# maxrmorrison/promonet

Hardware: AMD Instinct MI355X
Metric: audio samples/sec (22.05 kHz), batch-32 10 s utterances (higher is better)
Workload: dtype bf16; 1 GPU; Generator.forward (prepare_features + HiFi-GAN), batch 32 x 10 s per GPU (861 frames, 220416 samples each), random-init weights, bf16 MFMA operands, fp32 accumulate and activations; model=hifigan, batch_per_gpu=32, frames=861, devices=1, parallelism=batch-sharded x1

## Files before the change

### include/promonet_hip.h

```cpp
#ifndef PROMONET_HIP_H
#define PROMONET_HIP_H

#include <stddef.h>
#include <stdint.h>

#ifdef __cplusplus
extern "C" {
#endif

#define PM_OK 0
#define PM_EINVAL (-1)
#define PM_ESTATE (-2)
#define PM_EHIP (-3)
#define PM_ENOMEM (-4)
#define PM_ETIMEOUT (-5)

#define PM_F32 0
#define PM_F16 1
#define PM_BF16 2
#define PM_F16X3 3
#define PM_F16A2 4
#define PM_F16UX 5

#define PM_MAX_STAGES 8
// ... 49 lines not shown
                              void* stream);

int pm_hifigan_context(pm_hifigan_t h, int* left, int* right);
int pm_hifigan_stream(pm_hifigan_t h, const float* chunk, int chunk_cl,
                      int chunk_frames, const float* prev_window,
                      int prev_frames, int keep, float* next_window,
                      const float* global_features, int global_batch,
                      int emit_first, int emit_frames, float* out, int batch,
                      void* workspace, size_t workspace_bytes, void* stream);
size_t pm_hifigan_stream_workspace_bytes(pm_hifigan_t h, int batch,
                                         int window_frames);

int pm_hifigan_profile_enable(pm_hifigan_t h, int enable);
int pm_hifigan_profile_only(pm_hifigan_t h, const char* label);
int pm_hifigan_profile_collect(pm_hifigan_t h);
int pm_hifigan_profile_reset(pm_hifigan_t h);
const char* pm_hifigan_profile_report(pm_hifigan_t h);

#define PM_SPARSE_NONE 0
#define PM_SPARSE_PERCENTILE 1
#define PM_SPARSE_CONSTANT 2
#define PM_SPARSE_TOPK 3
int pm_prepare_features(const float* loudness, const float* pitch,
                        const float* periodicity, const float* ppg,
                        const float* pitch_edges, const float* pitch_table,
                        float* out_ref, float* out_cl, int batch, int frames,
                        int loudness_rows, int ppg_channels, int pitch_bins,
                        int embedding_size, int bands, int cl_channels,
                        int sparse_method, float ppg_threshold, float fmin,
                        float fmax, float min_db, float ref_db,
                        float period_rate, void* stream);

int pm_prepare_global_features(const int64_t* speakers,
                               const float* spectral_balance_ratios,
                               const float* loudness_ratios,
                               const float* speaker_table, float* out,
                               int batch, int speaker_channels,
                               int num_speakers, void* stream);
int pm_prepare_global_features_linear(const float* speaker_embeddings,
                                      const float* weight, const float* bias,
                                      const float* spectral_balance_ratios,
                                      const float* loudness_ratios,
                                      float* out, int batch,
                                      int embedding_channels,
                                      int speaker_channels, void* stream);

size_t pm_op_workspace_bytes(int c_in, int c_out, int k);
int pm_block_iteration_cl(int dtype, const float* x_cl, float* out_cl,
                          const float* w1, const float* b1, const float* w2,
                          const float* b2, int batch, int length,
                          int channels, int kernel_size, int dilation,
                          int mode, float scale, void* workspace,
                          size_t workspace_bytes, void* stream);
int pm_block_cl(int dtype, const float* x_cl, float* out_cl,
                const float* const* w1, const float* const* b1,
                const float* const* w2, const float* const* b2,
                const int* dilations, int niter, int batch, int length,
                int channels, int kernel_size, int mode, float scale,
                void* workspace, size_t workspace_bytes, void* stream);
int pm_block_act16_cl(int dtype, int act_dtype, const float* x_cl,
                      float* out_cl, void* act16_cl, const float* const* w1,
                      const float* const* b1, const float* const* w2,
                      const float* const* b2, const int* dilations, int niter,
                      int batch, int length, int channels, int kernel_size,
                      int mode, float scale, void* workspace,
                      size_t workspace_bytes, void* stream);
int pm_mrf_cl(int dtype, const float* x_cl, float* out_cl,
              const float* const* w1, const float* const* b1,
              const float* const* w2, const float* const* b2,
              const int* dilations, int niter, int batch, int length,
              int channels, void* workspace, size_t workspace_bytes,
              void* stream);
int pm_input_conv_cl(int dtype, const float* x_cl, float* out_cl,
                     const float* weight, const float* bias,
                     const float* global_features,
                     const float* speaker_weight, const float* speaker_bias,
                     int global_batch, int global_channels, int batch,
                     int length, int c_in, int c_out, void* workspace,
                     size_t workspace_bytes, void* stream);
int pm_conv_transpose_cl(int dtype, const float* x_cl, float* out_cl,
                         const float* w, const float* bias, int batch,
                         int length, int c_in, int c_out, int rate, int lrelu,
                         void* workspace, size_t workspace_bytes,
                         void* stream);
int pm_conv_transpose_ragged_cl(int dtype, const float* x_cl, float* out_cl,
                                const float* w, const float* bias,
                                const int* lengths, int batch, int length,
                                int c_in, int c_out, int rate, int lrelu,
                                void* workspace, size_t workspace_bytes,
                                void* stream);
int pm_conv_transpose_x16_cl(int dtype, const void* x16_cl, float* out_cl,
                             const float* w, const float* bias, int batch,
                             int length, int c_in, int c_out, int rate,
                             void* workspace, size_t workspace_bytes,
                             void* stream);
int pm_out_conv_tanh(const float* x_cl, const float* w, float* out,
                     int batch, int length, int channels, void* stream);
int pm_debug_timeline(void* dev_buffer);
int pm_debug_force(int walk_nseg, int upsample_groups);
int pm_debug_skew(int mode);
int pm_mfma_probe(int dtype, int iterations, const void* operands,
                  float* sink, int workgroups, void* stream);
size_t pm_walk_scratch_bytes(int batch);
int pm_fold_weight_norm(const float* g, const float* v, float* w, int rows,
                        int cols, void* stream);
int pm_to_channels_last(const float* src, float* dst, int batch, int channels,
// ... 336 lines not shown
```

### promonet_amd/_lib.py

```python
import ctypes
import os
from pathlib import Path

import torch

LIB_PATH = Path(__file__).parent / 'lib' / 'libpromonet_hip.so'

PM_F32, PM_F16, PM_BF16, PM_F16X3, PM_F16A2, PM_F16UX = 0, 1, 2, 3, 4, 5
DTYPES = {'fp32': PM_F32, 'f32': PM_F32, 'f16': PM_F16, 'fp16': PM_F16,
          'bf16': PM_BF16, 'f16x3': PM_F16X3, 'f16a2': PM_F16A2,
          'f16ux': PM_F16UX,
          'mixed': 16}
MAX_STAGES, MAX_RESBLOCKS, MAX_DILATIONS = 8, 4, 4
SPARSE_METHODS = {None: 0, 'percentile': 1, 'constant': 2, 'topk': 3}
DISC_SPEC_R, DISC_SPEC_CMB, DISC_SPEC_DB = range(3)
FDISC_ACTIVATIONS = {'none': 0, 'relu': 1, 'sigmoid': 2}
(ADV_ABS_DIFF, ADV_SQ_ONE_MINUS, ADV_SQ, ADV_HINGE_ONE_MINUS,
 ADV_HINGE_ONE_PLUS) = range(5)
(OPTIM_MAX, OPTIM_MIN, OPTIM_MEAN, OPTIM_NORM, OPTIM_NORM_SQ, OPTIM_NONFINITE,
 OPTIM_FOUND_INF, OPTIM_INV_SCALE, OPTIM_COEF) = range(9)
OPTIM_STATS = 16

c_float_p = ctypes.c_void_p
c_int64_p = ctypes.POINTER(ctypes.c_int64)


class HifiganConfig(ctypes.Structure):
    _fields_ = [
        ('num_features', ctypes.c_int),
        ('global_channels', ctypes.c_int),
        ('initial_channels', ctypes.c_int),
        ('num_stages', ctypes.c_int),
        ('upsample_rates', ctypes.c_int * MAX_STAGES),
        ('upsample_kernel_sizes', ctypes.c_int * MAX_STAGES),
        ('num_resblocks', ctypes.c_int),
        ('resblock_kernel_sizes', ctypes.c_int * MAX_RESBLOCKS),
        ('num_dilations', ctypes.c_int),
        ('resblock_dilations', (ctypes.c_int * MAX_DILATIONS) * MAX_RESBLOCKS),
        ('compute_dtype', ctypes.c_int),
        ('stage_compute_dtype', ctypes.c_int * MAX_STAGES)]


_I, _F, _P, _S = ctypes.c_int, ctypes.c_float, ctypes.c_void_p, ctypes.c_size_t
_D = ctypes.c_double
SIGNATURES = {
    'pm_version': (_I, []),
    'pm_last_error': (ctypes.c_char_p, []),
    'pm_hifigan_create': (_I, [ctypes.POINTER(HifiganConfig),
                               ctypes.POINTER(_P)]),
    'pm_hifigan_destroy': (_I, [_P]),
    'pm_hifigan_load_tensor': (_I, [_P, ctypes.c_char_p, _P, c_int64_p, _I, _P]),
    'pm_hifigan_finalize': (_I, [_P, _P]),
    'pm_hifigan_workspace_bytes': (_S, [_P, _I, _I]),
    'pm_hifigan_hopsize': (_I, [_P]),
    'pm_hifigan_features_cl_channels': (_I, [_P]),
    'pm_hifigan_forward': (_I, [_P, _P, _P, _I, _P, _I, _I, _P, _S, _P]),
    'pm_hifigan_forward_cl': (_I, [_P, _P, _P, _I, _P, _I, _I, _P, _S, _P]),
    'pm_hifigan_forward_ragged': (_I, [_P, _P, _I, _P, _I, _P, _P, _I, _I, _P, _S, _P]),
    'pm_hifigan_context': (_I, [_P, ctypes.POINTER(_I), ctypes.POINTER(_I)]),
    'pm_hifigan_stream': (_I, [_P, _P, _I, _I, _P, _I, _I, _P, _P, _I, _I, _I,
                               _P, _I, _P, _S, _P]),
    'pm_hifigan_stream_workspace_bytes': (_S, [_P, _I, _I]),
    'pm_hifigan_profile_enable': (_I, [_P, _I]),
    'pm_hifigan_profile_only': (_I, [_P, ctypes.c_char_p]),
    'pm_hifigan_profile_collect': (_I, [_P]),
    'pm_hifigan_profile_reset': (_I, [_P]),
    'pm_hifigan_profile_report': (ctypes.c_char_p, [_P]),
    'pm_prepare_features': (_I, [_P] * 8 + [_I] * 9 + [_F] * 6 + [_P]),
    'pm_prepare_global_features': (_I, [_P] * 5 + [_I, _I, _I, _P]),
    'pm_prepare_global_features_linear': (_I, [_P] * 6 + [_I, _I, _I, _P]),
    'pm_op_workspace_bytes': (_S, [_I, _I, _I]),
    'pm_block_iteration_cl': (_I, [_I] + [_P] * 6 + [_I] * 6 + [_F, _P, _S, _P]),
    'pm_block_cl': (_I, [_I, _P, _P] + [_P] * 5 + [_I] * 6 + [_F, _P, _S, _P]),
    'pm_block_act16_cl': (
        _I, [_I, _I, _P, _P, _P] + [_P] * 5 + [_I] * 6 + [_F, _P, _S, _P]),
    'pm_mrf_cl': (_I, [_I, _P, _P] + [_P] * 5 + [_I] * 4 + [_P, _S, _P]),
    'pm_input_conv_cl': (_I, [_I] + [_P] * 7 + [_I] * 6 + [_P, _S, _P]),
    'pm_conv_transpose_cl': (_I, [_I] + [_P] * 4 + [_I] * 6 + [_P, _S, _P]),
    'pm_conv_transpose_ragged_cl': (
        _I, [_I] + [_P] * 5 + [_I] * 6 + [_P, _S, _P]),
    'pm_conv_transpose_x16_cl': (_I, [_I] + [_P] * 4 + [_I] * 5 + [_P, _S, _P]),
    'pm_out_conv_tanh': (_I, [_P, _P, _P, _I, _I, _I, _P]),
    'pm_debug_timeline': (_I, [_P]),
    'pm_debug_force': (_I, [_I, _I]),
    'pm_debug_skew': (_I, [_I]),
    'pm_mfma_probe': (_I, [_I, _I, _P, _P, _I, _P]),
    'pm_walk_scratch_bytes': (_S, [_I]),
    'pm_fold_weight_norm': (_I, [_P, _P, _P, _I, _I, _P]),
    'pm_to_channels_last': (_I, [_P, _P, _I, _I, _I, _I, _P]),
    'pm_grid_sample': (_I, [_P, _P, _P, _I, _I, _I, _I, _F, _F, _F, _F, _P]),
    'pm_stretch_grid': (_I, [_P, _I, _P, _I, _P, _P, _I, _I, _P]),
    'pm_fargan_create': (_I, [_I, _I, _I, ctypes.POINTER(_P)]),
    'pm_fargan_destroy': (_I, [_P]),
    'pm_fargan_load_tensor': (_I, [_P, ctypes.c_char_p, _P, c_int64_p, _I, _P]),
    'pm_fargan_finalize': (_I, [_P, _P]),
    'pm_fargan_workspace_bytes': (_S, [_P, _I, _I]),
    'pm_fargan_forward': (_I, [_P, _P, _I, _P, _I, _P, _I, _P, _I, _I, _P, _S, _P]),
    'pm_fargan_forward_ragged': (_I, [_P, _P, _I, _P, _I, _P, _I, _P, _P, _I, _I, _P, _S, _P]),
    'pm_fargan_forward_stateful': (_I, [_P, _P, _I, _P, _I, _P, _I, _P, _P, _P, _P, _I, _I, _P, _S, _P]),
    'pm_fargan_set_mode': (_I, [_P, _I]),
    'pm_fargan_check': (_I, [_P, _I, _I, _P, _P]),
    'pm_stft_scratch_bytes': (_S, [_I, _I]),
    'pm_stft_magnitude': (_I, [_P, _P, _I, _I, _P, _S, _P]),
    'pm_stft_magnitude_dft': (_I, [_P, _P, _I, _I, _P, _S, _P]),
    'pm_stft_mel_scratch_bytes': (_S, [_I]),
    'pm_stft_mel_prepare': (_I, [_P, _I, _P, _S, _P]),
    'pm_stft_mel': (_I, [_P, _P, _P, _I, _I, _I, _I, _F, _P]),
    'pm_stft_set_frames_per_group': (_I, [_I]),
    'pm_stft_set_loudness_passes': (_I, [_I]),
    'pm_stft_launch_info': (_I, [_I, _I, _I, ctypes.POINTER(_I), ctypes.POINTER(_I)]),
    'pm_linear_to_mel': (_I, [_P, _P, _P, _I, _I, _I, _I, _I, _F, _P]),
    'pm_stft_backward_scratch_bytes': (_S, [_I, _I]),
    'pm_stft_magnitude_backward': (_I, [_P, _P, _P, _I, _I, _P, _S, _P]),
    'pm_linear_to_mel_backward': (_I, [_P] * 5 + [_I] * 5 + [_F, _P]),
    'pm_loudness_scratch_bytes': (_S, [_I, _I]),
    'pm_loudness': (_I, [_P, _P, _P, _I, _I, _I, _F, _P, _S, _P]),
    'pm_limit_tile': (_I, [ctypes.POINTER(_I), ctypes.POINTER(_I)]),
    'pm_limit_workspace_bytes': (_S, [_I]),
    'pm_limit': (_I, [_P] * 4 + [_I, _I, ctypes.c_int64, ctypes.c_int64, _I] +
                 [_F] * 4 + [_P, _S, _P]),
    'pm_loudness_shift': (_I, [_P] * 5 + [_I, _I, ctypes.c_int64, _I,
                                          ctypes.c_int64, ctypes.c_int64, _P]),
    'pm_resample_tile': (_I, [_I, _I, _I]),
    'pm_resample': (_I, [_P, _P, _P, _P, _I, _I, ctypes.c_int64, _I, _I, _I, _I,
                         ctypes.c_int64, _P]),
# ... 134 lines not shown
```

### promonet_amd/csrc/pm_api.hip

```cpp
#include <hip/hip_runtime.h>

#include <algorithm>
#include <cstdarg>
#include <cstdio>
#include <cstring>
#include <map>
#include <mutex>
#include <string>
#include <vector>

#include "pm_host.h"
#include "pm_launch.h"
#include "pm_misc.h"

#define PM_VERSION 100

static thread_local char g_error[512] = "";

int pm_fail(int code, const char* fmt, ...) {
    va_list ap;
    va_start(ap, fmt);
    vsnprintf(g_error, sizeof(g_error), fmt, ap);
    va_end(ap);
    return code;
// ... 973 lines not shown
    if (!speakers || !table || !out) return pm_fail(PM_EINVAL, "null argument");
    if (B < 1 || S < 1 || num_speakers < 1)
        return pm_fail(PM_EINVAL, "bad dimensions");
    hipLaunchKernelGGL(pm_global_features_kernel, dim3(B), dim3(256), 0,
                       (hipStream_t)stream, (const long long*)speakers, sbr,
                       lr, table, out, B, S, num_speakers);
    PM_HIP_TRY(hipGetLastError());
    return PM_OK;
}

extern "C" int pm_prepare_global_features_linear(
    const float* emb, const float* weight, const float* bias,
    const float* sbr, const float* lr, float* out, int B, int E, int S,
    void* stream) {
    if (!emb || !weight || !bias || !out)
        return pm_fail(PM_EINVAL, "null argument");
    if (B < 1 || E < 1 || S < 1) return pm_fail(PM_EINVAL, "bad dimensions");
    hipLaunchKernelGGL(pm_global_features_linear_kernel,
                       dim3((S + 3) / 4, B), dim3(256), 0,
                       (hipStream_t)stream, emb, weight, bias, sbr, lr, out, B,
                       E, S);
    PM_HIP_TRY(hipGetLastError());
    return PM_OK;
}

struct IterationLayout { float *w1, *w2, *b1, *b2; size_t total; };
static IterationLayout iteration_layout(int c_in, int c_out, int k,
                                        void* base) {
    const size_t ci = pm_pad32(c_in), co = pm_pad32(c_out);
    PmCarve c(base);
    return {c.take<float>(ci * co * k + co * 16),
            c.take<float>(ci * co * k + co * 16), c.take<float>(co * 64),
            c.take<float>(co * 64), c.used};
}

extern "C" size_t pm_op_workspace_bytes(int c_in, int c_out, int k) {
    return iteration_layout(c_in, c_out, k, nullptr).total;
}

static int pack_iteration(
    int dtype, int C, int K, const float* w1, const float* b1, const float* w2,
    const float* b2, char* base, hipStream_t s, const void** p1,
    const void** p2) {
    const IterationLayout l = iteration_layout(C, C, K, base);
    Layer conv = mrf_layer(dtype, C, K);
    conv.w = l.w1; conv.bias = l.b1;
    PM_HIP_TRY(pack_layer(conv, w1, b1, s));
    conv.w = l.w2; conv.bias = l.b2;
    PM_HIP_TRY(pack_layer(conv, w2, b2, s));
    *p1 = l.w1; *p2 = l.w2;
    return PM_OK;
}

extern "C" int pm_block_iteration_cl(
    int dtype, const float* x, float* out, const float* w1, const float* b1,
    const float* w2, const float* b2, int B, int L, int C, int K, int d,
    int mode, float scale, void* ws, size_t ws_bytes, void* stream) {
    if (!x || !out || !w1 || !b1 || !w2 || !b2 || !ws)
        return pm_fail(PM_EINVAL, "null argument");
    const int Cp = pm_pad32(C);
    if (Cp != 32 && Cp != 64 && Cp != 128 && Cp != 256)
        return pm_fail(PM_EINVAL, "channels %d unsupported", C);
    if ((K != 3 && K != 7 && K != 11) || d < 1 || d > 5)
        return pm_fail(PM_EINVAL, "kernel %d / dilation %d unsupported", K, d);
    if (ws_bytes < pm_op_workspace_bytes(C, C, K))
        return pm_fail(PM_ENOMEM, "workspace too small");
    hipStream_t s = (hipStream_t)stream;
    const void *p1, *p2;
    const int rc = pack_iteration(dtype, C, K, w1, b1, w2, b2, (char*)ws, s,
                                  &p1, &p2);
    if (rc) return rc;
    PairArgs a = {};
    a.x = x; a.out = out; a.w1 = p1; a.w2 = p2;
    a.B = B; a.L = L; a.dilation = d; a.mode = mode; a.scale = scale;
    PM_HIP_TRY(launch_pair(dtype, Cp, K, a, s));
    return PM_OK;
}

extern "C" int pm_debug_timeline(void* dev_buffer) {
#ifdef PM_TUNING
    g_timeline = (unsigned long long*)dev_buffer;
    return PM_OK;
#else
    (void)dev_buffer;
    return pm_fail(PM_ESTATE, "pm_debug_timeline needs a -DPM_TUNING build "
                              "(make TUNING=1)");
#endif
}

static int block_cl_impl(
    int dtype, const float* x, float* out, const float* const* w1,
    const float* const* b1, const float* const* w2, const float* const* b2,
    const int* dilations, int niter, int B, int L, int C, int K, int mode,
    float scale, void* ws, size_t ws_bytes, void* stream, void* act16,
    int act_dtype) {
    if (!x || !out || !w1 || !b1 || !w2 || !b2 || !dilations || !ws)
        return pm_fail(PM_EINVAL, "null argument");
    const int Cp = pm_pad32(C);
    if (Cp > 256)
        return pm_fail(PM_EINVAL, "channels %d unsupported (<= 256)", C);
    if ((K != 3 && K != 7 && K != 11) || niter < 1 || niter > 3)
        return pm_fail(PM_EINVAL,
                       "kernel %d / %d iterations unsupported", K, niter);
    const size_t per = iteration_layout(C, C, K, nullptr).total;
    if (ws_bytes < 3 * per)
        return pm_fail(PM_ENOMEM, "workspace too small");
    hipStream_t s = (hipStream_t)stream;
    PmStage d = stage_desc(Cp, x, out, B, L, mode, scale, 1, niter);
    d.blk[0].K = K;
    for (int n = 0; n < niter; ++n) {
        const int rc = pack_iteration(dtype, C, K, w1[n], b1[n], w2[n], b2[n],
                                      (char*)ws + n * per, s, &d.blk[0].w1[n],
                                      &d.blk[0].w2[n]);
        if (rc) return rc;
        d.blk[0].dil[n] = dilations[n];
    }
    if (ws_bytes > 3 * per) {
        d.scratch = (char*)ws + 3 * per;
        d.scratch_bytes = ws_bytes - 3 * per;
    }
    if (act16) { d.act16 = act16; d.act16_type = act_dtype; }
    PmPlan plan;
    PM_HIP_TRY(plan_stage(dtype, d, 1, &plan));
    if (plan.block[0].kernel == PM_PAIRS)
        return pm_fail(PM_EINVAL, "no whole-Block kernel for this shape");
    PM_HIP_TRY(launch_block3(dtype, plan.block[0], d, 0, s));
    if (act16 && !plan.block[0].act16)
        return pm_fail(PM_ESTATE,
                       "the launch did not take the skewed walk: `out` "
// ... 292 lines not shown
```

### promonet_amd/csrc/pm_conv.h

```cpp
#pragma once
#include <type_traits>

#include "pm_common.h"


template <class ET, int CH, int NT, int XR_MAX>
struct ChunkStager {
    static constexpr int Q = CH / 4;
    static constexpr int MAXIT = (XR_MAX * Q + NT - 1) / NT;
    static constexpr int S = CH * ET::ESZ + 16;
    float4 r[MAXIT];

    __device__ __forceinline__ void load(
        const float* __restrict__ xb, int cstride, int c0, int t_first,
        int XR, int L, int tid) {
        const int lo = max(t_first, 0);
        const int hi = min(L, t_first + XR);
        const __amdgpu_buffer_rsrc_t rsrc = __builtin_amdgcn_make_buffer_rsrc(
            const_cast<float*>(xb) + (size_t)lo * cstride, 0,
            max(hi - lo, 0) * cstride * 4, 0x00020000);
#pragma unroll
        for (int it = 0; it < MAXIT; ++it) {
            const int idx = tid + it * NT;
            const int row = idx / Q, q = idx % Q;
// ... 341 lines not shown
#pragma unroll
        for (int g4 = 0; g4 < 4; g4 += 2) {
            float4 lo = pm_lrelu4(acc_quad(v, g4));
            float4 hi = pm_lrelu4(acc_quad(v, g4 + 1));
            if (MASK && zero) {
                lo = make_float4(0.f, 0.f, 0.f, 0.f);
                hi = lo;
            }
            uint2 a = ET::pack4(lo), b = ET::pack4(hi);
            auto sx = __builtin_amdgcn_permlane32_swap(a.x, b.x, false, false);
            auto sy = __builtin_amdgcn_permlane32_swap(a.y, b.y, false, false);
            *reinterpret_cast<uint4*>(rowp + (ch + 8 * (g4 + lh)) * 2) =
                make_uint4(sx[0], sy[0], sx[1], sy[1]);
        }
    } else if constexpr (ET::SPLIT && !PM_SPLIT_STORE8) {
#pragma unroll
        for (int g4 = 0; g4 < 4; ++g4) {
            float4 q = pm_lrelu4(acc_quad(v, g4));
            if (MASK && zero) q = make_float4(0.f, 0.f, 0.f, 0.f);
            half4 hi, lo;
            ElemF16X3::split4(q, hi, lo);
            const uint2 a = __builtin_bit_cast(uint2, hi);
            const uint2 b = __builtin_bit_cast(uint2, lo);
            auto sx = __builtin_amdgcn_permlane32_swap(a.x, b.x, false, false);
            auto sy = __builtin_amdgcn_permlane32_swap(a.y, b.y, false, false);
            *reinterpret_cast<uint4*>(rowp + ((ch >> 3) + g4) * 32 + lh * 16) =
                make_uint4(sx[0], sy[0], sx[1], sy[1]);
        }
    } else {
#pragma unroll
        for (int g4 = 0; g4 < 4; ++g4) {
            float4 q = pm_lrelu4(acc_quad(v, g4));
            if (MASK && zero) q = make_float4(0.f, 0.f, 0.f, 0.f);
            ET::store4_at(rowp, ch + 8 * g4 + 4 * lh, q);
        }
    }
}

template <class ET>
__device__ __forceinline__ void store_tile_lrelu(
    char* rowp, const int ch, const floatx16& v, const int t_tile,
    const int L, const int ln, const int lh) {
#if defined(PM_TUNING) && defined(PM_ABLATE_EPI)
    return;
#endif
    if (t_tile >= 0 && t_tile + 32 <= L) {
        store_tile_lrelu_impl<ET, false>(rowp, ch, v, false, lh);
    } else {
        const int t = t_tile + ln;
        store_tile_lrelu_impl<ET, true>(rowp, ch, v, !(t >= 0 && t < L), lh);
    }
}


struct PairArgs {
    const float* x;
    float* out;
    const void* w1;
    const void* w2;
    int B, L;
    int dilation;
    int mode;
    float scale;
    int ntiles;
    const int* lengths;
    int len_scale;
    PM_TIMELINE_FIELD
};

template <int C, int K, int WN, int NTW>
struct PairGeom {
    static constexpr int N1 = WN * NTW * 32;
    static constexpr int TL = N1 - (K - 1);
};

template <class ET, int C, int K, int WM, int WN, int NTW, int CH, int ALIAS>
__host__ __device__ constexpr int pair_smem_bytes(int d) {
    constexpr int NCH = C / CH;
    constexpr int N1 = WN * NTW * 32;
    const int x = (NCH > 1 ? 2 : 1) * (N1 + (K - 1) * d) * (CH * ET::ESZ + 16);
    const int inter = (N1 + K - 1) * (C * ET::ESZ + 16);
    return ALIAS ? (x > inter ? x : inter) : x + inter;
}

template <class ET, int C, int K, int WM, int WN, int NTW, int CH, int ALIAS>
__global__ __launch_bounds__(WM * WN * 64) void conv_pair_kernel(
    PairArgs a) {
    typedef typename ET::afrag_t frag_t;
    constexpr int NCH = C / CH;
    constexpr int KC = CH / 16;
    constexpr int MT = C / 32;
    constexpr int MTW = MT / WM;
    static_assert(MT % WM == 0, "WM must divide the M tile count");
    constexpr int N1 = WN * NTW * 32;
    constexpr int NT = WM * WN * 64;
    constexpr int H2 = (K - 1) / 2;
    constexpr int TL = N1 - (K - 1);
    constexpr int SX = CH * ET::ESZ + 16;
    constexpr int SI = C * ET::ESZ + 16;
    constexpr int XR_MAX = N1 + (K - 1) * 5;
    constexpr int G = (ET::ESZ == 4) ? (KC >= 2 ? 2 : 1)
                    : (KC < 4 ? KC : (NTW >= 6 && K == 11 ? 2 : 4));

    extern __shared__ __attribute__((aligned(16))) char smem[];

    const int tid = threadIdx.x;
// ... 65 lines not shown
        if (more) {
            pm_block_sync();
            if (c < 2) PM_STAMP(a, 8 + 3 * c);
        }
    }

    PM_STAMP(a, 2);
    if (ALIAS) pm_block_sync();
    load_bias_frags<ET, MTW>(bf, w2 + W_BIAS, W_MT_STRIDE);
#pragma unroll
    for (int mt = 0; mt < MTW; ++mt) {
#pragma unroll
        for (int nt = 0; nt < NTW; ++nt) {
            const int n_first = (wn * NTW + nt) * 32;
            const int n = n_first + ln;
            const int t_tile = t0 - H2 + n_first;
            store_tile_lrelu<ET>(inter + n * SI, (wm * MTW + mt) * 32,
                                 acc[mt][nt], t_tile, L, ln, lh);
            const int t = min(t0 + n, L - 1);
            const float* xr = xb + (size_t)t * C +
                              (wm * MTW + mt) * 32 + 4 * lh;
#pragma unroll
            for (int g4 = 0; g4 < 4; ++g4) {
                const float4 r = *reinterpret_cast<const float4*>(xr + 8 * g4);
                acc[mt][nt][4 * g4 + 0] = r.x;
                acc[mt][nt][4 * g4 + 1] = r.y;
                acc[mt][nt][4 * g4 + 2] = r.z;
                acc[mt][nt][4 * g4 + 3] = r.w;
            }
        }
    }
    pm_block_sync();
    __builtin_amdgcn_sched_barrier(0);
    bias_add<ET, MTW, NTW>(acc, bf);
    PM_STAMP(a, 3);

    const int lane_off_i = ((wn * NTW * 32) + ln) * SI + lh * 8 * ET::ESZ;
#pragma unroll 1
    for (int c = 0; c < NCH; ++c) {
        mma_taps<ET, K, KC, MTW, NTW, G, SI>(
            acc, inter + lane_off_i + c * CH * ET::ESZ, SI,
            w2 + (size_t)c * W_CHUNK, W_MT_STRIDE, afirst,
            c + 1 < NCH ? w2 + (size_t)(c + 1) * W_CHUNK : nullptr);
    }

    PM_STAMP(a, 4);
    const int mode = a.mode;
    const float scale = a.scale;
    const int rows = min(TL, L - t0);
    const __amdgpu_buffer_rsrc_t orsrc = __builtin_amdgcn_make_buffer_rsrc(
        a.out + ((size_t)b * a.L + t0) * C, 0, rows * C * 4, 0x00020000);
    const unsigned voff0 =
        (unsigned)(((wn * NTW * 32 + ln) * C + wm * MTW * 32 + 4 * lh) * 4);
    if (mode == 2) {
        constexpr int NB = NTW > 4 ? (NTW + 1) / 2 : NTW;
#pragma unroll
        for (int mt = 0; mt < MTW; ++mt)
#pragma unroll
            for (int n0 = 0; n0 < NTW; n0 += NB) {
                pm_u4 old[NB][4];
#pragma unroll
                for (int i = 0; i < NB; ++i) {
                    if (n0 + i >= NTW) break;
                    const unsigned voff =
                        voff0 + (unsigned)((mt * 32 + (n0 + i) * 32 * C) * 4);
#pragma unroll
                    for (int g4 = 0; g4 < 4; ++g4)
                        old[i][g4] = __builtin_amdgcn_raw_buffer_load_b128(
                            orsrc, voff + g4 * 32, 0, 0);
                }
#pragma unroll
                for (int i = 0; i < NB; ++i) {
                    if (n0 + i >= NTW) break;
                    const int nt = n0 + i;
                    const unsigned voff =
                        voff0 + (unsigned)((mt * 32 + nt * 32 * C) * 4);
#pragma unroll
                    for (int g4 = 0; g4 < 4; ++g4) {
                        const pm_u4 o = old[i][g4];
                        pm_u4 r;
                        r.x = __float_as_uint(__uint_as_float(o.x) +
                                              acc[mt][nt][4 * g4 + 0] * scale);
                        r.y = __float_as_uint(__uint_as_float(o.y) +
                                              acc[mt][nt][4 * g4 + 1] * scale);
                        r.z = __float_as_uint(__uint_as_float(o.z) +
                                              acc[mt][nt][4 * g4 + 2] * scale);
                        r.w = __float_as_uint(__uint_as_float(o.w) +
                                              acc[mt][nt][4 * g4 + 3] * scale);
                        __builtin_amdgcn_raw_buffer_store_b128(
                            r, orsrc, voff + g4 * 32, 0, 0);
                    }
                }
            }
    } else {
        const float s = mode == 1 ? scale : 1.f;
#pragma unroll
        for (int mt = 0; mt < MTW; ++mt)
#pragma unroll
            for (int nt = 0; nt < NTW; ++nt) {
                const unsigned voff =
                    voff0 + (unsigned)((mt * 32 + nt * 32 * C) * 4);
#pragma unroll
                for (int g4 = 0; g4 < 4; ++g4) {
                    pm_u4 r;
                    r.x = __float_as_uint(acc[mt][nt][4 * g4 + 0] * s);
                    r.y = __float_as_uint(acc[mt][nt][4 * g4 + 1] * s);
                    r.z = __float_as_uint(acc[mt][nt][4 * g4 + 2] * s);
                    r.w = __float_as_uint(acc[mt][nt][4 * g4 + 3] * s);
                    __builtin_amdgcn_raw_buffer_store_b128(
                        r, orsrc, voff + g4 * 32, 0, 0);
                }
            }
    }
    PM_STAMP(a, 5);
    PM_STAMP_WALL(a, blockIdx.x, 13);
}


#ifndef PM_ROWS_AUX
#define PM_ROWS_AUX 2
#endif
#ifndef PM_SINGLE_ROWS
#define PM_SINGLE_ROWS 1
#endif
template <int MTW, int CP>
struct RowStores {
    static constexpr int RUN = MTW * 32 * 4;
    static constexpr int WAVE = CP * RUN;
    static constexpr int LPR = RUN / 16;
    static constexpr int CPI = 64 / LPR;
    static_assert(MTW == 1 || MTW == 2, "8 or 16 slots of 16 bytes");
    static_assert(CP == 8 || CP == 16 || CP == 32, "whole 8-lane store groups");
    static __device__ __forceinline__ int at(int col, int s) {
        return col * RUN + ((s ^ (col & 7)) << 4);
    }
};

template <int MTW, int NTW, int CP>
__device__ __forceinline__ void pm_store_rows(
    const floatx16 (&acc)[MTW][NTW], char* ebuf, const float* bias_ptr,
    const float* gb, __amdgpu_buffer_rsrc_t orsrc, int M, int m0, int n0,
    int lane) {
    typedef RowStores<MTW, CP> R;
    const int ln = lane & 31, lh = lane >> 5;
    const int q = lane % R::LPR, h = lane / R::LPR;
    const int co = m0 + 4 * q;
    float4 bias = *reinterpret_cast<const float4*>(bias_ptr + co);
    if (gb) {
        const float4 g = *reinterpret_cast<const float4*>(gb + co);
        bias.x += g.x; bias.y += g.y; bias.z += g.z; bias.w += g.w;
    }
#pragma unroll
    for (int pass = 0; pass < NTW * (32 / CP); ++pass) {
        const int nt = pass / (32 / CP), sub = pass % (32 / CP);
        pm_wave_lds_sync();
        if (CP == 32 || ln / CP == sub) {
#pragma unroll
            for (int mt = 0; mt < MTW; ++mt)
#pragma unroll
                for (int g4 = 0; g4 < 4; ++g4)
                    *reinterpret_cast<float4*>(
                        ebuf + R::at(ln % CP, mt * 8 + 2 * g4 + lh)) =
                        make_float4(acc[mt][nt][4 * g4 + 0],
                                    acc[mt][nt][4 * g4 + 1],
                                    acc[mt][nt][4 * g4 + 2],
                                    acc[mt][nt][4 * g4 + 3]);
        }
        pm_wave_lds_sync();
        const int n = n0 + nt * 32 + sub * CP + h;
        const unsigned voff = (unsigned)((n * M + co) * 4);
#pragma unroll
        for (int k = 0; k < CP / R::CPI; ++k) {
            const float4 v = *reinterpret_cast<const float4*>(
                ebuf + R::at(R::CPI * k + h, q));
            pm_u4 r;
            r.x = __float_as_uint(v.x + bias.x);
            r.y = __float_as_uint(v.y + bias.y);
            r.z = __float_as_uint(v.z + bias.z);
            r.w = __float_as_uint(v.w + bias.w);
            __builtin_amdgcn_raw_buffer_store_b128(
                r, orsrc, voff + (unsigned)(k * R::CPI * M * 4), 0,
                PM_ROWS_AUX);
        }
    }
}

struct SingleArgs {
    const void* x16;
    const float* x;
    float* out;
    const void* w;
    const float* bias;
    const float* gbias;
    int gbias_batch;
    int B, L, Cin, M;
    int Lout;
    int bins;
    unsigned* maxbits;
    const float* grad;
    int lrelu;
    int pad;
    int phase_c, phase_p, phase_r;
    int ntiles, nmblocks;
    const int* lengths;
    int len_scale;
};

__device__ __forceinline__ unsigned pm_float_order_bits(float f) {
    const unsigned u = __float_as_uint(f);
    return (u & 0x80000000u) ? ~u : (u | 0x80000000u);
}

template <class ET, int KT, int KSPAN, int CH, int WM, int WN, int MTW, int NTW,
          int EPI>
__global__ __launch_bounds__(WM * WN * 64) void conv_single_kernel(
    SingleArgs a) {
    typedef typename ET::afrag_t frag_t;
    constexpr int KC = CH / 16;
    constexpr int N1 = WN * NTW * 32;
    constexpr int NT = WM * WN * 64;
    constexpr int SX = CH * ET::ESZ + 16;
    constexpr int XR = N1 + KSPAN - 1;
    constexpr int MB = WM * MTW * 32;
    constexpr int G = (ET::ESZ == 4) ? (KC >= 2 ? 2 : 1) : KC;

    extern __shared__ __attribute__((aligned(16))) char smem[];

    const int tid = threadIdx.x;
    const int lane = tid & 63;
    const int wave = tid >> 6;
    const int wm = wave / WN, wn = wave % WN;
    const int ln = lane & 31, lh = lane >> 5;

    const int wg = pm_xcd_remap(blockIdx.x, gridDim.x);
    const int mb = wg % a.nmblocks;
    const int tile = (wg / a.nmblocks) % a.ntiles;
    const int b = wg / (a.nmblocks * a.ntiles);
    const int t0 = tile * N1;
// ... 614 lines not shown
            for (int nt = 0; nt < NTW; ++nt) {
                if (!last) {
                    const int col_first = (wn * NTW + nt) * 32;
                    const int col = col_first + ln2;
                    const int t_tile = c_first + col_first;
                    store_tile_lrelu<ET>(abuf + (MA + col) * S,
                                         m_first + mt * 32, trunk[mt][nt],
                                         t_tile, L, ln2, lh2);
                }
            }
        if (!last) bias_start<ET, MTW, NTW>(acc, bf);
        if (!last) pm_block_sync();
        PM_STAMP(a, 5 + 4 * it);
    }

    if constexpr (XMODE & 2) {
#pragma unroll
        for (int mt = 0; mt < MTW; ++mt)
#pragma unroll
            for (int nt = 0; nt < NTW; ++nt) xnext[mt][nt] = acc[mt][nt];
    }
    if constexpr (SUM == 1 || SUM == 2) {
#pragma unroll
        for (int mt = 0; mt < MTW; ++mt)
#pragma unroll
            for (int nt = 0; nt < NTW; ++nt) {
                if (SUM == 1) sum[mt][nt] = trunk[mt][nt];
                else sum[mt][nt] += trunk[mt][nt];
            }
        return;
    }
    if constexpr (SUM == 3) {
#pragma unroll
        for (int mt = 0; mt < MTW; ++mt)
#pragma unroll
            for (int nt = 0; nt < NTW; ++nt) trunk[mt][nt] += sum[mt][nt];
    }
#if defined(PM_TUNING) && defined(PM_ABLATE_OUT)
    if (trunk[0][0][0] != 12345.f) return;
#endif
    const int mode = SUM == 3 ? 1 : a.mode;
    const float scale = a.scale;
    const int own_first = c_first + store_lo;
    const __amdgpu_buffer_rsrc_t orsrc = __builtin_amdgcn_make_buffer_rsrc(
        a.out + ((size_t)b * a.L + own_first) * C, 0,
        max(min(store_n, L - own_first), 0) * C * 4, 0x00020000);
    int tid_s = tid;
    if constexpr (WALK) asm volatile("" : "+v"(tid_s));
    const int lane_s = tid_s & 63;
    const int wave_s = __builtin_amdgcn_readfirstlane(tid_s >> 6);
    const unsigned ovoff0 = (unsigned)(
        (((wave_s % WN) * NTW * 32 + (lane_s & 31) - store_lo) * C +
         (wave_s / WN) * MTW * 32 + 4 * (lane_s >> 5)) * 4);
    if (mode == 2) {
        constexpr int NB = NTW > 4 ? (NTW + 1) / 2 : NTW;
#pragma unroll
        for (int mt = 0; mt < MTW; ++mt)
#pragma unroll
            for (int n0 = 0; n0 < NTW; n0 += NB) {
                pm_u4 old[NB][4];
#pragma unroll
                for (int i = 0; i < NB; ++i) {
                    if (n0 + i >= NTW) break;
                    const unsigned voff = ovoff0 +
                        (unsigned)((mt * 32 + (n0 + i) * 32 * C) * 4);
#pragma unroll
                    for (int g4 = 0; g4 < 4; ++g4)
                        old[i][g4] = __builtin_amdgcn_raw_buffer_load_b128(
                            orsrc, voff + g4 * 32, 0, 0);
                }
#pragma unroll
                for (int i = 0; i < NB; ++i) {
                    if (n0 + i >= NTW) break;
                    const int nt = n0 + i;
                    const unsigned voff =
                        ovoff0 + (unsigned)((mt * 32 + nt * 32 * C) * 4);
#pragma unroll
                    for (int g4 = 0; g4 < 4; ++g4) {
                        const pm_u4 o = old[i][g4];
                        pm_u4 r;
                        r.x = __float_as_uint(__uint_as_float(o.x) +
                                              trunk[mt][nt][4 * g4 + 0] * scale);
                        r.y = __float_as_uint(__uint_as_float(o.y) +
                                              trunk[mt][nt][4 * g4 + 1] * scale);
                        r.z = __float_as_uint(__uint_as_float(o.z) +
                                              trunk[mt][nt][4 * g4 + 2] * scale);
                        r.w = __float_as_uint(__uint_as_float(o.w) +
                                              trunk[mt][nt][4 * g4 + 3] * scale);
                        __builtin_amdgcn_raw_buffer_store_b128(
                            r, orsrc, voff + g4 * 32, 0, 0);
                    }
                }
            }
    } else {
        const float sc = mode == 1 ? scale : 1.f;
#pragma unroll
        for (int mt = 0; mt < MTW; ++mt)
#pragma unroll
            for (int nt = 0; nt < NTW; ++nt) {
                const unsigned voff =
                    ovoff0 + (unsigned)((mt * 32 + nt * 32 * C) * 4);
#pragma unroll
                for (int g4 = 0; g4 < 4; ++g4) {
                    pm_u4 r;
                    r.x = __float_as_uint(trunk[mt][nt][4 * g4 + 0] * sc);
                    r.y = __float_as_uint(trunk[mt][nt][4 * g4 + 1] * sc);
                    r.z = __float_as_uint(trunk[mt][nt][4 * g4 + 2] * sc);
                    r.w = __float_as_uint(trunk[mt][nt][4 * g4 + 3] * sc);
// ... 565 lines not shown
                        (2 * H2 + wn * NTW * 32 + (te & 63)) * S +
                        m_first * ET::ESZ;
#pragma unroll
                    for (int mt = 0; mt < MTW; ++mt)
#pragma unroll
                        for (int g4 = 0; g4 < 4; ++g4) {
                            const float4 v = *reinterpret_cast<const float4*>(
                                slot + mt * 32 * ET::ESZ + g4 * 16);
                            trunk[mt][0][4 * g4 + 0] = v.x;
                            trunk[mt][0][4 * g4 + 1] = v.y;
                            trunk[mt][0][4 * g4 + 2] = v.z;
                            trunk[mt][0][4 * g4 + 3] = v.w;
                        }
                } else {
                    const unsigned xi =
                        (unsigned)((((par ^ 1) * 2 + it) * WM + wm) * GE::TB) +
                        dead;
#pragma unroll
                    for (int mt = 0; mt < MTW; ++mt)
#pragma unroll
                        for (int g4 = 0; g4 < 4; ++g4) {
                            const pm_u4 v = __builtin_amdgcn_raw_buffer_load_b128(
                                srsrc, xi + lane_slot + mt * 4096 + g4 * 1024, 0,
                                AUX);
                            trunk[mt][0][4 * g4 + 0] = __uint_as_float(v.x);
                            trunk[mt][0][4 * g4 + 1] = __uint_as_float(v.y);
                            trunk[mt][0][4 * g4 + 2] = __uint_as_float(v.z);
                            trunk[mt][0][4 * g4 + 3] = __uint_as_float(v.w);
                        }
                }
            }
        }

        const int o = c0 - skew;
        const int ts = fresh_tid();
        const int ln = ts & 31, lh = (ts >> 5) & 1;
        const int own_first = max(s0, o);
        const int own_n = min(e0, o + NC) - own_first;
        const float scale = a.scale;
        const int mode = a.mode;
        const __amdgpu_buffer_rsrc_t orsrc = __builtin_amdgcn_make_buffer_rsrc(
            a.out + ((size_t)b * a.L + own_first) * C, 0,
            max(own_n, 0) * C * 4, 0x00020000);
        const unsigned ovoff0 = (unsigned)(
            ((o - own_first + wn * NTW * 32 + ln) * C + m_first + 4 * lh) * 4);
        const bool a16 = a.act16 != nullptr;
        const bool a16f = a.act16_type == 1;
        const __amdgpu_buffer_rsrc_t arsrc = __builtin_amdgcn_make_buffer_rsrc(
            reinterpret_cast<char*>(a.act16) +
                ((size_t)b * a.L + own_first) * C * 2, 0,
            a16 ? max(own_n, 0) * C * 2 : 0, 0x00020000);
        const float sc = mode == 0 ? 1.f : scale;
        constexpr int NB = MTW * NTW < 4 ? MTW * NTW : 4;
#pragma unroll
        for (int t0 = 0; t0 < MTW * NTW; t0 += NB) {
            pm_u4 old[NB][4] = {};
            if (mode == 2) {
#pragma unroll
                for (int i = 0; i < NB; ++i) {
                    if (t0 + i >= MTW * NTW) break;
                    const int mt = (t0 + i) / NTW, nt = (t0 + i) % NTW;
                    const unsigned voff =
                        ovoff0 + (unsigned)((mt * 32 + nt * 32 * C) * 4);
#pragma unroll
                    for (int g4 = 0; g4 < 4; ++g4)
                        old[i][g4] = __builtin_amdgcn_raw_buffer_load_b128(
                            orsrc, voff + g4 * 32, 0, 0);
                }
            }
#pragma unroll
            for (int i = 0; i < NB; ++i) {
                if (t0 + i >= MTW * NTW) break;
                const int mt = (t0 + i) / NTW, nt = (t0 + i) % NTW;
                const unsigned voff =
                    ovoff0 + (unsigned)((mt * 32 + nt * 32 * C) * 4);
                float4 rq[4];
#pragma unroll
                for (int g4 = 0; g4 < 4; ++g4)
                    rq[g4] = make_float4(
                        __uint_as_float(old[i][g4].x) +
                            trunk[mt][nt][4 * g4 + 0] * sc,
                        __uint_as_float(old[i][g4].y) +
                            trunk[mt][nt][4 * g4 + 1] * sc,
                        __uint_as_float(old[i][g4].z) +
                            trunk[mt][nt][4 * g4 + 2] * sc,
                        __uint_as_float(old[i][g4].w) +
                            trunk[mt][nt][4 * g4 + 3] * sc);
                if (a16) {
                    const unsigned v16 = (voff - 16u * lh) / 2;
#pragma unroll
                    for (int g4 = 0; g4 < 4; g4 += 2) {
                        const float4 lo = pm_lrelu4(rq[g4]);
                        const float4 hi = pm_lrelu4(rq[g4 + 1]);
                        const uint2 pa = a16f ? ElemF16::pack4(lo)
                                              : ElemBF16::pack4(lo);
                        const uint2 pb = a16f ? ElemF16::pack4(hi)
                                              : ElemBF16::pack4(hi);
                        auto sx = __builtin_amdgcn_permlane32_swap(
                            pa.x, pb.x, false, false);
                        auto sy = __builtin_amdgcn_permlane32_swap(
                            pa.y, pb.y, false, false);
                        const pm_u4 u = {sx[0], sy[0], sx[1], sy[1]};
                        __builtin_amdgcn_raw_buffer_store_b128(
                            u, arsrc, v16 + 16 * (g4 + lh), 0, 0);
                    }
                } else {
// ... 505 lines not shown
```

Before: 401.3 million samples/s.

## Stage residual-block output tiles through LDS for coalesced row stores

Adds a row-store epilogue for 16-bit residual-block kernels (pair, whole-block, skewed). The MFMA accumulators go through a swizzled LDS buffer so each lane writes contiguous 16-byte channel runs per row, covering the residual add, scaling, and optional fused leaky-ReLU to a 16-bit activation buffer. The aim is to replace scattered per-fragment global stores and loads with coalesced row accesses, at the cost of extra LDS traffic and wave syncs. It also adds a ragged-length block-iteration API entry point.

```diff
diff --git a/include/promonet_hip.h b/include/promonet_hip.h
--- a/include/promonet_hip.h
+++ b/include/promonet_hip.h
@@ -125,6 +125,13 @@
                           int channels, int kernel_size, int dilation,
                           int mode, float scale, void* workspace,
                           size_t workspace_bytes, void* stream);
+int pm_block_iteration_ragged_cl(int dtype, const float* x_cl, float* out_cl,
+                                 const float* w1, const float* b1,
+                                 const float* w2, const float* b2,
+                                 const int* lengths, int batch, int length,
+                                 int channels, int kernel_size, int dilation,
+                                 int mode, float scale, void* workspace,
+                                 size_t workspace_bytes, void* stream);
 int pm_block_cl(int dtype, const float* x_cl, float* out_cl,
                 const float* const* w1, const float* const* b1,
                 const float* const* w2, const float* const* b2,
diff --git a/promonet_amd/_lib.py b/promonet_amd/_lib.py
--- a/promonet_amd/_lib.py
+++ b/promonet_amd/_lib.py
@@ -71,6 +71,8 @@
     'pm_prepare_global_features_linear': (_I, [_P] * 6 + [_I, _I, _I, _P]),
     'pm_op_workspace_bytes': (_S, [_I, _I, _I]),
     'pm_block_iteration_cl': (_I, [_I] + [_P] * 6 + [_I] * 6 + [_F, _P, _S, _P]),
+    'pm_block_iteration_ragged_cl': (
+        _I, [_I] + [_P] * 7 + [_I] * 6 + [_F, _P, _S, _P]),
     'pm_block_cl': (_I, [_I, _P, _P] + [_P] * 5 + [_I] * 6 + [_F, _P, _S, _P]),
     'pm_block_act16_cl': (
         _I, [_I, _I, _P, _P, _P] + [_P] * 5 + [_I] * 6 + [_F, _P, _S, _P]),
diff --git a/promonet_amd/csrc/pm_api.hip b/promonet_amd/csrc/pm_api.hip
--- a/promonet_amd/csrc/pm_api.hip
+++ b/promonet_amd/csrc/pm_api.hip
@@ -1049,10 +1049,11 @@
     return PM_OK;
 }
 
-extern "C" int pm_block_iteration_cl(
+static int block_iteration_cl_impl(
     int dtype, const float* x, float* out, const float* w1, const float* b1,
-    const float* w2, const float* b2, int B, int L, int C, int K, int d,
-    int mode, float scale, void* ws, size_t ws_bytes, void* stream) {
+    const float* w2, const float* b2, const int* lengths, int B, int L, int C,
+    int K, int d, int mode, float scale, void* ws, size_t ws_bytes,
+    void* stream) {
     if (!x || !out || !w1 || !b1 || !w2 || !b2 || !ws)
         return pm_fail(PM_EINVAL, "null argument");
     const int Cp = pm_pad32(C);
@@ -1070,8 +1071,29 @@
     PairArgs a = {};
     a.x = x; a.out = out; a.w1 = p1; a.w2 = p2;
     a.B = B; a.L = L; a.dilation = d; a.mode = mode; a.scale = scale;
+    a.lengths = lengths; a.len_scale = 1;
     PM_HIP_TRY(launch_pair(dtype, Cp, K, a, s));
     return PM_OK;
+}
+
+extern "C" int pm_block_iteration_cl(
+    int dtype, const float* x, float* out, const float* w1, const float* b1,
+    const float* w2, const float* b2, int B, int L, int C, int K, int d,
+    int mode, float scale, void* ws, size_t ws_bytes, void* stream) {
+    return block_iteration_cl_impl(dtype, x, out, w1, b1, w2, b2, nullptr, B,
+                                   L, C, K, d, mode, scale, ws, ws_bytes,
+                                   stream);
+}
+
+extern "C" int pm_block_iteration_ragged_cl(
+    int dtype, const float* x, float* out, const float* w1, const float* b1,
+    const float* w2, const float* b2, const int* lengths, int B, int L, int C,
+    int K, int d, int mode, float scale, void* ws, size_t ws_bytes,
+    void* stream) {
+    if (!lengths) return pm_fail(PM_EINVAL, "null argument");
+    return block_iteration_cl_impl(dtype, x, out, w1, b1, w2, b2, lengths, B,
+                                   L, C, K, d, mode, scale, ws, ws_bytes,
+                                   stream);
 }
 
 extern "C" int pm_debug_timeline(void* dev_buffer) {
diff --git a/promonet_amd/csrc/pm_conv.h b/promonet_amd/csrc/pm_conv.h
--- a/promonet_amd/csrc/pm_conv.h
+++ b/promonet_amd/csrc/pm_conv.h
@@ -417,6 +417,187 @@
     }
 }
 
+#ifndef PM_ROWS_AUX
+#define PM_ROWS_AUX 2
+#endif
+#ifndef PM_SINGLE_ROWS
+#define PM_SINGLE_ROWS 1
+#endif
+template <int MTW, int CP>
+struct RowStores {
+    static constexpr int RUN = MTW * 32 * 4;
+    static constexpr int WAVE = CP * RUN;
+    static constexpr int LPR = RUN / 16;
+    static constexpr int CPI = 64 / LPR;
+    static_assert(MTW == 1 || MTW == 2, "8 or 16 slots of 16 bytes");
+    static_assert(CP == 8 || CP == 16 || CP == 32, "whole 8-lane store groups");
+    static __device__ __forceinline__ int at(int col, int s) {
+        return col * RUN + ((s ^ (col & 7)) << 4);
+    }
+};
+
+template <int MTW, int NTW, int CP>
+__device__ __forceinline__ void pm_store_rows(
+    const floatx16 (&acc)[MTW][NTW], char* ebuf, const float* bias_ptr,
+    const float* gb, __amdgpu_buffer_rsrc_t orsrc, int M, int m0, int n0,
+    int lane) {
+    typedef RowStores<MTW, CP> R;
+    const int ln = lane & 31, lh = lane >> 5;
+    const int q = lane % R::LPR, h = lane / R::LPR;
+    const int co = m0 + 4 * q;
+    float4 bias = *reinterpret_cast<const float4*>(bias_ptr + co);
+    if (gb) {
+        const float4 g = *reinterpret_cast<const float4*>(gb + co);
+        bias.x += g.x; bias.y += g.y; bias.z += g.z; bias.w += g.w;
+    }
+#pragma unroll
+    for (int pass = 0; pass < NTW * (32 / CP); ++pass) {
+        const int nt = pass / (32 / CP), sub = pass % (32 / CP);
+        pm_wave_lds_sync();
+        if (CP == 32 || ln / CP == sub) {
+#pragma unroll
+            for (int mt = 0; mt < MTW; ++mt)
+#pragma unroll
+                for (int g4 = 0; g4 < 4; ++g4)
+                    *reinterpret_cast<float4*>(
+                        ebuf + R::at(ln % CP, mt * 8 + 2 * g4 + lh)) =
+                        make_float4(acc[mt][nt][4 * g4 + 0],
+                                    acc[mt][nt][4 * g4 + 1],
+                                    acc[mt][nt][4 * g4 + 2],
+                                    acc[mt][nt][4 * g4 + 3]);
+        }
+        pm_wave_lds_sync();
+        const int n = n0 + nt * 32 + sub * CP + h;
+        const unsigned voff = (unsigned)((n * M + co) * 4);
+#pragma unroll
+        for (int k = 0; k < CP / R::CPI; ++k) {
+            const float4 v = *reinterpret_cast<const float4*>(
+                ebuf + R::at(R::CPI * k + h, q));
+            pm_u4 r;
+            r.x = __float_as_uint(v.x + bias.x);
+            r.y = __float_as_uint(v.y + bias.y);
+            r.z = __float_as_uint(v.z + bias.z);
+            r.w = __float_as_uint(v.w + bias.w);
+            __builtin_amdgcn_raw_buffer_store_b128(
+                r, orsrc, voff + (unsigned)(k * R::CPI * M * 4), 0,
+                PM_ROWS_AUX);
+        }
+    }
+}
+
+#ifndef PM_OUT_ROWS
+#define PM_OUT_ROWS 7
+#endif
+#ifndef PM_OUT_ROWS_AUX
+#define PM_OUT_ROWS_AUX 2
+#endif
+#ifndef PM_OUT_ROWS_K11
+#define PM_OUT_ROWS_K11 0
+#endif
+template <int MTW, int NTW, int NB, bool ZADD, bool A16>
+__device__ __forceinline__ void pm_store_out_rows(
+    const floatx16 (&acc)[MTW][NTW], char* ebuf, __amdgpu_buffer_rsrc_t orsrc,
+    int C, int m0, int n0, int mode, float scale, int lane,
+    __amdgpu_buffer_rsrc_t arsrc, bool a16, bool a16f) {
+    typedef RowStores<MTW, 32> R;
+    constexpr int KI = 32 / R::CPI;
+    const int ln = lane & 31, lh = lane >> 5;
+    const int q = lane % R::LPR, h = lane / R::LPR;
+    const int q8 = lane % (R::LPR / 2), h8 = lane / (R::LPR / 2);
+    const unsigned voff0 = (unsigned)(((n0 + h) * C + m0 + 4 * q) * 4);
+    const unsigned voff8 = (unsigned)(((n0 + h8) * C + m0 + 8 * q8) * 4);
+    const float s = mode == 0 ? 1.f : scale;
+    const bool wide = A16 && a16;
+#pragma unroll
+    for (int p0 = 0; p0 < NTW; p0 += NB) {
+        pm_u4 old[NB][KI] = {};
+        if (mode == 2) {
+#pragma unroll
+            for (int i = 0; i < NB; ++i) {
+                if (p0 + i >= NTW) break;
+                const unsigned col = (unsigned)((p0 + i) * 32 * C * 4);
+#pragma unroll
+                for (int k = 0; k < KI; ++k)
+                    old[i][k] = __builtin_amdgcn_raw_buffer_load_b128(
+                        orsrc,
+                        wide ? voff8 + col +
+                                   (unsigned)((k / 2) * 2 * R::CPI * C * 4 +
+                                              (k % 2) * 16)
+                             : voff0 + col + (unsigned)(k * R::CPI * C * 4),
+                        0, 0);
+            }
+        }
+#pragma unroll
+        for (int i = 0; i < NB; ++i) {
+            if (p0 + i >= NTW) break;
+            const int nt = p0 + i;
+            const unsigned col = (unsigned)(nt * 32 * C * 4);
+            pm_wave_lds_sync();
+#pragma unroll
+            for (int mt = 0; mt < MTW; ++mt)
+#pragma unroll
+                for (int g4 = 0; g4 < 4; ++g4)
+                    *reinterpret_cast<float4*>(
+                        ebuf + R::at(ln, mt * 8 + 2 * g4 + lh)) =
+                        acc_quad(acc[mt][nt], g4);
+            pm_wave_lds_sync();
+            if (wide) {
+                if constexpr (A16) {
+#pragma unroll
+                    for (int k = 0; k < KI; k += 2) {
+                        const int c8 = R::CPI * k + h8;
+                        float4 rq[2];
+#pragma unroll
+                        for (int j = 0; j < 2; ++j) {
+                            const float4 v = *reinterpret_cast<const float4*>(
+                                ebuf + R::at(c8, 2 * q8 + j));
+                            const pm_u4 o = old[i][k + j];
+                            rq[j] = make_float4(
+                                __uint_as_float(o.x) + v.x * s,
+                                __uint_as_float(o.y) + v.y * s,
+                                __uint_as_float(o.z) + v.z * s,
+                                __uint_as_float(o.w) + v.w * s);
+                        }
+                        const float4 lo = pm_lrelu4(rq[0]);
+                        const float4 hi = pm_lrelu4(rq[1]);
+                        const uint2 pa = a16f ? ElemF16::pack4(lo)
+                                              : ElemBF16::pack4(lo);
+                        const uint2 pb = a16f ? ElemF16::pack4(hi)
+                                              : ElemBF16::pack4(hi);
+                        const pm_u4 u = {pa.x, pa.y, pb.x, pb.y};
+                        __builtin_amdgcn_raw_buffer_store_b128(
+                            u, arsrc,
+                            (voff8 + col + (unsigned)(k * R::CPI * C * 4)) / 2,
+                            0, PM_OUT_ROWS_AUX);
+                    }
+                }
+            } else {
+#pragma unroll
+                for (int k = 0; k < KI; ++k) {
+                    const float4 v = *reinterpret_cast<const float4*>(
+                        ebuf + R::at(R::CPI * k + h, q));
+                    const pm_u4 o = old[i][k];
+                    pm_u4 r;
+                    if (ZADD || mode == 2) {
+                        r.x = __float_as_uint(__uint_as_float(o.x) + v.x * s);
+                        r.y = __float_as_uint(__uint_as_float(o.y) + v.y * s);
+                        r.z = __float_as_uint(__uint_as_float(o.z) + v.z * s);
+                        r.w = __float_as_uint(__uint_as_float(o.w) + v.w * s);
+                    } else {
+                        r.x = __float_as_uint(v.x * s);
+                        r.y = __float_as_uint(v.y * s);
+                        r.z = __float_as_uint(v.z * s);
+                        r.w = __float_as_uint(v.w * s);
+                    }
+                    __builtin_amdgcn_raw_buffer_store_b128(
+                        r, orsrc, voff0 + col + (unsigned)(k * R::CPI * C * 4),
+                        0, PM_OUT_ROWS_AUX);
+                }
+            }
+        }
+    }
+}
+
 
 struct PairArgs {
     const float* x;
@@ -588,8 +769,20 @@
         a.out + ((size_t)b * a.L + t0) * C, 0, rows * C * 4, 0x00020000);
     const unsigned voff0 =
         (unsigned)(((wn * NTW * 32 + ln) * C + wm * MTW * 32 + 4 * lh) * 4);
-    if (mode == 2) {
-        constexpr int NB = NTW > 4 ? (NTW + 1) / 2 : NTW;
+    constexpr int NB = NTW > 4 ? (NTW + 1) / 2 : NTW;
+    constexpr bool OUT_ROWS =
+        (PM_OUT_ROWS & 1) && ET::ESZ == 2 && MTW == 1 &&
+        pair_smem_bytes<ET, C, K, WM, WN, NTW, CH, ALIAS>(1) >=
+            WM * WN * MTW * 4096;
+    static_assert(OUT_ROWS || !(PM_OUT_ROWS & 1) || ET::ESZ != 2,
+                  "a 16-bit pair geometry lost the row stores");
+    if constexpr (OUT_ROWS) {
+        pm_block_sync();
+        pm_store_out_rows<MTW, NTW, NB, false, false>(
+            acc, smem + wave * RowStores<MTW, 32>::WAVE, orsrc, C,
+            wm * MTW * 32, wn * NTW * 32, mode, scale, lane, orsrc, false,
+            false);
+    } else if (mode == 2) {
 #pragma unroll
         for (int mt = 0; mt < MTW; ++mt)
 #pragma unroll
@@ -652,74 +845,6 @@
     PM_STAMP_WALL(a, blockIdx.x, 13);
 }
 
-
-#ifndef PM_ROWS_AUX
-#define PM_ROWS_AUX 2
-#endif
-#ifndef PM_SINGLE_ROWS
-#define PM_SINGLE_ROWS 1
-#endif
-template <int MTW, int CP>
-struct RowStores {
-    static constexpr int RUN = MTW * 32 * 4;
-    static constexpr int WAVE = CP * RUN;
-    static constexpr int LPR = RUN / 16;
-    static constexpr int CPI = 64 / LPR;
-    static_assert(MTW == 1 || MTW == 2, "8 or 16 slots of 16 bytes");
-    static_assert(CP == 8 || CP == 16 || CP == 32, "whole 8-lane store groups");
-    static __device__ __forceinline__ int at(int col, int s) {
-        return col * RUN + ((s ^ (col & 7)) << 4);
-    }
-};
-
-template <int MTW, int NTW, int CP>
-__device__ __forceinline__ void pm_store_rows(
-    const floatx16 (&acc)[MTW][NTW], char* ebuf, const float* bias_ptr,
-    const float* gb, __amdgpu_buffer_rsrc_t orsrc, int M, int m0, int n0,
-    int lane) {
-    typedef RowStores<MTW, CP> R;
-    const int ln = lane & 31, lh = lane >> 5;
-    const int q = lane % R::LPR, h = lane / R::LPR;
-    const int co = m0 + 4 * q;
-    float4 bias = *reinterpret_cast<const float4*>(bias_ptr + co);
-    if (gb) {
-        const float4 g = *reinterpret_cast<const float4*>(gb + co);
-        bias.x += g.x; bias.y += g.y; bias.z += g.z; bias.w += g.w;
-    }
-#pragma unroll
-    for (int pass = 0; pass < NTW * (32 / CP); ++pass) {
-        const int nt = pass / (32 / CP), sub = pass % (32 / CP);
-        pm_wave_lds_sync();
-        if (CP == 32 || ln / CP == sub) {
-#pragma unroll
-            for (int mt = 0; mt < MTW; ++mt)
-#pragma unroll
-                for (int g4 = 0; g4 < 4; ++g4)
-                    *reinterpret_cast<float4*>(
-                        ebuf + R::at(ln % CP, mt * 8 + 2 * g4 + lh)) =
-                        make_float4(acc[mt][nt][4 * g4 + 0],
-                                    acc[mt][nt][4 * g4 + 1],
-                                    acc[mt][nt][4 * g4 + 2],
-                                    acc[mt][nt][4 * g4 + 3]);
-        }
-        pm_wave_lds_sync();
-        const int n = n0 + nt * 32 + sub * CP + h;
-        const unsigned voff = (unsigned)((n * M + co) * 4);
-#pragma unroll
-        for (int k = 0; k < CP / R::CPI; ++k) {
-            const float4 v = *reinterpret_cast<const float4*>(
-                ebuf + R::at(R::CPI * k + h, q));
-            pm_u4 r;
-            r.x = __float_as_uint(v.x + bias.x);
-            r.y = __float_as_uint(v.y + bias.y);
-            r.z = __float_as_uint(v.z + bias.z);
-            r.w = __float_as_uint(v.w + bias.w);
-            __builtin_amdgcn_raw_buffer_store_b128(
-                r, orsrc, voff + (unsigned)(k * R::CPI * M * 4), 0,
-                PM_ROWS_AUX);
-        }
-    }
-}
 
 struct SingleArgs {
     const void* x16;
@@ -1440,8 +1565,17 @@
     const unsigned ovoff0 = (unsigned)(
         (((wave_s % WN) * NTW * 32 + (lane_s & 31) - store_lo) * C +
          (wave_s / WN) * MTW * 32 + 4 * (lane_s >> 5)) * 4);
-    if (mode == 2) {
-        constexpr int NB = NTW > 4 ? (NTW + 1) / 2 : NTW;
+    constexpr int NB = NTW > 4 ? (NTW + 1) / 2 : NTW;
+    constexpr bool OUT_ROWS = (PM_OUT_ROWS & 4) && ET::ESZ == 2 && MTW == 1 &&
+                              ROWS_A * S >= WM * WN * MTW * 4096;
+    static_assert(OUT_ROWS || !(PM_OUT_ROWS & 4) || ET::ESZ != 2,
+                  "a 16-bit whole-Block geometry lost the row stores");
+    if constexpr (OUT_ROWS) {
+        pm_store_out_rows<MTW, NTW, NB, false, false>(
+            trunk, abuf + wave_s * RowStores<MTW, 32>::WAVE, orsrc, C,
+            (wave_s / WN) * MTW * 32, (wave_s % WN) * NTW * 32 - store_lo,
+            mode, scale, lane_s, orsrc, false, false);
+    } else if (mode == 2) {
 #pragma unroll
         for (int mt = 0; mt < MTW; ++mt)
 #pragma unroll
@@ -2113,6 +2247,19 @@
             a16 ? max(own_n, 0) * C * 2 : 0, 0x00020000);
         const float sc = mode == 0 ? 1.f : scale;
         constexpr int NB = MTW * NTW < 4 ? MTW * NTW : 4;
+        constexpr bool OUT_ROWS = (PM_OUT_ROWS & 2) && ET::ESZ == 2 &&
+                                  MTW == 1 && (K != 11 || PM_OUT_ROWS_K11) &&
+                                  GE::RT * S >= WM * WN * MTW * 4096;
+        static_assert(OUT_ROWS || !(PM_OUT_ROWS & 2) || ET::ESZ != 2 ||
+                          (K == 11 && !PM_OUT_ROWS_K11),
+                      "a 16-bit skewed geometry lost the row stores");
+        if constexpr (OUT_ROWS) {
+            pm_block_sync();
+            pm_store_out_rows<MTW, NTW, NB, true, true>(
+                trunk, tbuf + wave * RowStores<MTW, 32>::WAVE, orsrc, C,
+                m_first, o - own_first + wn * NTW * 32, mode, scale, ts & 63,
+                arsrc, a16, a16f);
+        } else
 #pragma unroll
         for (int t0 = 0; t0 < MTW * NTW; t0 += NB) {
             pm_u4 old[NB][4] = {};
```

Result: faster. 408.5 million samples/s, median of 6 (+1.8%).
